# Princic-1837592/julia-raytracer

Measured on AMD Instinct MI355X. Metric: Mrays/s + wall-clock render time, cornellbox 1280×720×256spp, higher is better.
Workload: dtype f32; 1 GPU; cornellbox path 1280x720x256spp; scene=cornellbox, sampler=path, width=1280, height=720, spp=256, bounces=8, batch=256, traversal=near, traversal_requested=auto, bvh=middle, parallelism=1 tile groups x 1 sample ranges + RCCL reduce

## Files before the change

### julia-raytracer_amd/csrc/jt_integrator.h

```cpp
#pragma once

#include <hip/hip_runtime.h>

#include "jt_bsdf.h"
#include "jt_device.h"
#include "jt_launch.h"
#include "jt_scene_eval.h"
#include "jt_traverse.h"

#ifndef JT_FUSED_BSDF
#define JT_FUSED_BSDF 1
#endif

namespace jtk {
using namespace jtd;

template <int F>
__device__ __forceinline__ v3 sample_lights(const DScene& S, v3 position, float rl, float rel, v2 ruv) {
    const int light_id = sample_uniform(S.nlights, rl);
    const DLight l = S.lights[light_id - 1];
    const float* cdf = S.cdf + l.cdf_offset;
    if (l.instance >= 0) {
        const int element = l.nguide ? sample_discrete_guided(cdf, l.ncdf, rel, S.guide_t + l.guide_offset,
                                                              S.guide_a + l.guide_offset, l.nguide, l.guide_scale)
// ... 191 lines not shown
}
template <int F>
__device__ __forceinline__ bool light_hit(const DScene& S, const DParams& P, Path& st, const Hit& h) {
    if (h.hit && light_hit_add<F>(S, st, h)) return false;
    return light_chain_end<F>(S, P, st);
}

#ifndef JT_LIGHT_LEAF_STEP
#define JT_LIGHT_LEAF_STEP 1
#endif
#ifndef JT_CHAIN_TAIL
#define JT_CHAIN_TAIL 2
#endif
__host__ __device__ constexpr bool ft_mesh_kernel(int F) { return mesh_family(F); }
template <bool WIDE, int F>
__host__ __device__ constexpr bool chain_tail() {
    return JT_CHAIN_TAIL && !WIDE && !(F & FT_NOIL) && F != FT_NONE && !ft_mesh_kernel(F);
}
template <bool WIDE, bool OVF, bool NCACHE, int F>
__host__ __device__ constexpr bool chain_leaf_step() {
    return JT_LIGHT_LEAF_STEP && !WIDE && !OVF && !NCACHE && !ft_mesh_kernel(F);
}
template <bool WIDE, bool OVF, bool NCACHE, int F>
__host__ __device__ constexpr bool chain_dinv_once() {
    return JT_CHAIN_TAIL >= 2 && chain_tail<WIDE, F>() && chain_leaf_step<WIDE, OVF, NCACHE, F>();
}

template <bool WIDE, int RING, bool OVF, int COUNT, bool NCACHE, int F, class CountLq>
__device__ __forceinline__ bool light_chain(const DScene& S, const DParams& P, Path& st, Trav& T, int* stack, int pixel,
                                            Counters& cnt, CountLq count_lq) {
    constexpr bool RERUN_LOOP = ft_mesh_kernel(F);
    constexpr bool LEAF = chain_leaf_step<WIDE, OVF, NCACHE, F>(), TAIL = chain_tail<WIDE, F>();
    constexpr bool DINV_ONCE = chain_dinv_once<WIDE, OVF, NCACHE, F>();
    const auto dinv = [&] { T.wdinv = V3(jl_rcp(st.d.x), jl_rcp(st.d.y), jl_rcp(st.d.z)); };
    const auto query = [&] {
        count_lq();
        const int inst = S.lights[st.li].instance;
        if (LEAF) {
            if (!DINV_ONCE) dinv();
            const int negmask = DINV_ONCE && !(F & FT_XFORM) ? T.negmask : neg_mask(st.d, S.order_flip);
            inst_leaf_query<COUNT, F>(S, T, st.o, st.d, T.wdinv, negmask, inst, cnt);
            while (T.nprim > 0) prim_step<COUNT, F>(S, T, cnt);
        } else {
            query_start<WIDE>(S, T, st.o, st.d, inst, stack);
            do {
                node_step_any<WIDE, RING, OVF, COUNT, NCACHE, F>(S, T, stack, pixel, cnt);
                while (T.nprim > 0) prim_step<COUNT, F>(S, T, cnt);
            } while (RERUN_LOOP && rerun_tie<WIDE>(S, T, st.o, st.d, inst, stack));
        }
    };
    if (TAIL) {
        if (DINV_ONCE) {
            dinv();
            if (!(F & FT_XFORM)) T.negmask = neg_mask(st.d, S.order_flip);
        }
        for (;;) {
            do query();
            while (T.h_inst >= 0 && light_hit_add<F>(S, st, query_hit(T)));
            if (light_chain_end<F>(S, P, st)) return true;
            if (st.phase != PH_LIGHT) return false;
        }
    }
    do {
        query();
        if (light_hit<F>(S, P, st, query_hit(T))) return true;
    } while (st.phase == PH_LIGHT);
    return false;
}

struct Aov {
    float* acc;
    float w_;
    int first_;
    int lk_;
    template <int F>
    __device__ __forceinline__ float w() const {
        if (!lane_lds(F)) return w_;
        if (ft_none(F)) return 1.0f / (float)(((reinterpret_cast<const int*>(acc)[11 * BLOCK] - first_) >> lk_) + 1);
        return acc[12 * BLOCK];
    }
};
template <int F>
__device__ __forceinline__ void aov_update(const Aov& a, v3 ta, v3 tn) {
    const float aw = a.w<F>();
    const float omw = 1 - aw;
    float* p = a.acc;
    p[4 * BLOCK] = p[4 * BLOCK] * omw + ta.x * aw;
// ... 206 lines not shown
```

### julia-raytracer_amd/csrc/jt_kernels.h

```cpp
#pragma once

#include <hip/hip_runtime.h>

#include <algorithm>

#include "jt_integrator.h"
#include "jt_launch.h"

namespace jtk {
using namespace jtd;

#ifndef JT_STAMPS
#define JT_STAMPS 0
#endif
#ifndef JT_NODE_REPEAT_NONE
#define JT_NODE_REPEAT_NONE 4
#endif
#ifndef JT_NODE_REPEAT
#define JT_NODE_REPEAT 3
#endif
#ifndef JT_FIRST_POP_NONE
#define JT_FIRST_POP_NONE 1
#endif
#ifndef JT_FIRST_POP
// ... 101 lines not shown
    return JT_ITEM_FIRST_POP == 1 || (JT_ITEM_FIRST_POP == 2 && !WIDE && !ft_none(F));
}
constexpr unsigned ITEM_NONE = 0xffffffffu;

__device__ __forceinline__ int item_pixel(unsigned item, const DParams& P, int tiles_x) {
    const int t = (int)(item >> 6), l = (int)(item & 63u);
    return ((t / tiles_x) * 8 + (l >> 3)) * P.width + (t % tiles_x) * 8 + (l & 7);
}
__host__ __device__ __forceinline__ int item_slot(unsigned item, const DParams& P) {
    const int t = (int)(item >> 6);
    float inv = 1.0f / (float)P.tile_stride;
#if defined(__HIP_DEVICE_COMPILE__)
    inv = __uint_as_float(__builtin_amdgcn_readfirstlane(__float_as_uint(inv)));
#endif
    const int u = (int)((float)(t - P.tile_offset) * inv + 0.5f);
    return u * 64 + (int)(item & 63u);
}
__device__ __forceinline__ float stream_weight(const DParams& P, int s) {
    return 1.0f / (float)(((s - P.first) >> P.lk) + 1);
}

#if JT_STAMPS
#define JT_STAMP(x) x
#else
#define JT_STAMP(x)
#endif

template <int SAMPLER, int RING, bool OVF, int COUNT, int F, bool NCACHE, bool WIDE>
__device__ __forceinline__ void trace_body_items(const DScene& S0, const DParams& P0, int s_begin, int s_end,
                                                 const DAccum& A, int* stack) {
    const DScene& S = S0;
    const DParams& P = P0;
    static_assert(lane_lds(F), "the per-lane item body keeps the lane's sample index in LDS");
    const int lane = threadIdx.x & 63;
    const int oslot = (int)blockIdx.x * BLOCK + (int)threadIdx.x;
    if constexpr ((F & (FT_TEX | FT_ENV)) != 0) {
        for (int k = threadIdx.x; k < 512; k += BLOCK) tex_lut[k] = k < 256 ? S.srgb_lut[k] : S.byte_lut[k - 256];
        __syncthreads();
    }
    Counters cnt{0, 0, 0, 0};
    constexpr bool WC = !ft_none(F);
    unsigned w_paths = 0, w_rays = 0, w_lq = 0;
    __shared__ unsigned wave_cnt[WC ? 1 : (BLOCK / 64) * 4];
    unsigned* const wcnt = wave_cnt + (WC ? 0 : (threadIdx.x >> 6) * 4);
    if (!WC && lane < 3) wcnt[lane] = 0u;
    auto lds_count = [&](int k, bool c) {
        if (c) __hip_atomic_fetch_add(wcnt + k, 1u, __ATOMIC_RELAXED, __HIP_MEMORY_SCOPE_WORKGROUP);
    };
    __shared__ float acc_lds[acc_slots(F) * BLOCK];
    float* acc = acc_lds + threadIdx.x;
    int* const acc_i = reinterpret_cast<int*>(acc);
#if JT_STAMPS
    unsigned long long t_trav = 0, t_shade = 0, n_trav = 0, n_shade = 0, lanes_p = 0, lanes_n = 0, steps_p = 0, steps_n = 0;
    unsigned long long t_hit = 0, t_fin = 0, t_qb = 0, n_phit = 0, n_fin = 0, idle = 0, n_mph = 0, n_mty = 0, n_mid = 0;
    unsigned long long lanes_sh = 0, lanes_hit = 0, t_start = 0, n_start = 0, lanes_start = 0;
#endif
    const int tiles_x = (P.width + 7) / 8, tiles = launch_tiles(P);
    const int kstr = 1 << P.lk;
    const int nq = s_end - s_begin < kstr ? s_end - s_begin : kstr;
    unsigned xcc;
    asm volatile("s_getreg_b32 %0, hwreg(HW_REG_XCC_ID)" : "=s"(xcc));
    int band_k = 0;
    int ut = 0, uq = 0, bnext = 64;
    bool drained = false;
    unsigned item = ITEM_NONE;
    bool next_sample = false;
// ... 56 lines not shown
                            nr = JT_A(normal)[pixel];
                            h = (int)JT_A(hits)[pixel];
                        } else {
                            const size_t o = (size_t)((s - P.first) & (kstr - 1)) * (size_t)JT_A(nslot) +
                                             (size_t)item_slot(item, P);
                            im = JT_A(part_img)[o];
                            al = JT_A(part_alb)[o];
                            nr = JT_A(part_nrm)[o];
                            h = __float_as_int(al.w);
                        }
                    }
                    acc[0] = im.x;
                    acc[BLOCK] = im.y;
                    acc[2 * BLOCK] = im.z;
                    acc[3 * BLOCK] = im.w;
                    acc[4 * BLOCK] = al.x;
                    acc[5 * BLOCK] = al.y;
                    acc[6 * BLOCK] = al.z;
                    acc[7 * BLOCK] = nr.x;
                    acc[8 * BLOCK] = nr.y;
                    acc[9 * BLOCK] = nr.z;
                    acc_i[10 * BLOCK] = h;
                }
            }
            bnext += take;
        }
        next_sample = false;
        if (start) {
            const int sample = acc_i[11 * BLOCK];
            const int pixel = item_pixel(item, P, tiles_x);
            if (!ft_none(F)) acc[12 * BLOCK] = stream_weight(P, sample);
            const DParams& P = karg_params<karg_params_on<SAMPLER, F>()>(P0);
            start_path<F>(P, pixel % P.width, pixel / P.width, pixel, sample, st);
            query_start<WIDE>(S, T, st.o, st.d, -1, stack);
            if (!WC) lds_count(1, true);
            if constexpr (item_first_pop<WIDE, F>()) {
#pragma unroll
                for (int k = 0; k < first_pops<F>(); k++)
                    if (wants_node<WIDE>(T)) node_step_any<WIDE, RING, OVF, COUNT, NCACHE, F>(S, T, stack, oslot, cnt);
            }
        }
        if (WC) w_rays += lane_count(__builtin_amdgcn_ballot_w64(start));
#if JT_STAMPS
        const unsigned long long ts1 = __builtin_amdgcn_s_memtime();
        t_start += ts1 - ts0;
        n_start++;
        lanes_start += lane_count(__builtin_amdgcn_ballot_w64(start));
#endif
        if (__builtin_amdgcn_ballot_w64(item != ITEM_NONE) == 0) break;
        constexpr bool LSTEP = light_steps(SAMPLER, F);
        for (;;) {
            const bool wantp = T.nprim > 0;
            const bool wantn = wants_node<WIDE>(T);
            const bool waiting = query_done<WIDE>(T);
            const int np = lane_count(__builtin_amdgcn_ballot_w64(wantp));
            const int nn = lane_count(__builtin_amdgcn_ballot_w64(wantn));
            int nw = lane_count(__builtin_amdgcn_ballot_w64(waiting));
            const int nb = np + nn;
            if (LSTEP && !S.light_inline) {
                const bool wantl = waiting && st.phase == PH_LIGHT;
                const int nl = lane_count(__builtin_amdgcn_ballot_w64(wantl));
                if (nl > 0 && (nl >= P.light_lanes || nb == 0)) {
                    bool c_lq = false, c_ray = false;
                    if (wantl && rerun_tie<WIDE>(S, T, st.o, st.d, S.lights[st.li].instance, stack)) {
                    } else if (wantl) {
                        if (light_hit<F>(S, P, st, query_hit(T))) {
                            st.phase = PH_FINISH;
                        } else if (st.phase == PH_LIGHT) {
                            if (WC) c_lq = true;
                            else lds_count(2, true);
                            query_start<WIDE>(S, T, st.o, st.d, S.lights[st.li].instance, stack);
                        } else {
                            if (WC) c_ray = true;
                            else lds_count(1, true);
                            query_start<WIDE>(S, T, st.o, st.d, -1, stack);
                        }
                    }
                    if (WC) {
                        w_lq += lane_count(__builtin_amdgcn_ballot_w64(c_lq));
                        w_rays += lane_count(__builtin_amdgcn_ballot_w64(c_ray));
                    }
                    continue;
                }
                nw -= nl;
            }
            if (nb == 0 || nw >= (nb + nw < P.wait_lanes ? nb + nw : P.wait_lanes)) break;
#if JT_STAMPS
            n_trav++;
            idle += 64 - lane_count(__builtin_amdgcn_ballot_w64(item != ITEM_NONE));
            if (np * JT_VOTE_P >= nn * JT_VOTE_N) { steps_p++; lanes_p += np; } else { steps_n++; lanes_n += nn; }
#endif
            if (JT_RAY_FROM_PATH && !(F & FT_XFORM)) {
                T.lo = st.o;
                T.ld = st.d;
            }
            if (np * JT_VOTE_P >= nn * JT_VOTE_N) {
                if (T.nprim > 0) prim_step<COUNT, F>(S, T, cnt);
            } else {
                constexpr int NREP = ft_none(F) ? JT_NODE_REPEAT_NONE : JT_NODE_REPEAT;
#pragma unroll
                for (int k = 0; k < NREP; k++)
                    if (wants_node<WIDE>(T)) node_step_any<WIDE, RING, OVF, COUNT, NCACHE, F>(S, T, stack, oslot, cnt);
            }
        }
#if JT_STAMPS
        const unsigned long long ts2 = __builtin_amdgcn_s_memtime();
        t_trav += ts2 - ts1;
        n_shade++;
        lanes_sh += lane_count(__builtin_amdgcn_ballot_w64(query_done<WIDE>(T)));
        {
            int mid = -1, mt = -1;
            if (query_done<WIDE>(T) && st.phase == PH_SCENE && T.h_inst >= 0) {
                mid = S.inst_shade[T.h_inst].material;
                mt = (F & FT_MAT) ? S.materials[mid].type : (int)M_MATTE;
            }
            if (__builtin_amdgcn_ballot_w64(mt >= 0)) {
                n_mph++;
                lanes_hit += lane_count(__builtin_amdgcn_ballot_w64(mt >= 0));
                for (int ty = 0; ty <= (int)M_GLTFPBR; ty++) n_mty += __builtin_amdgcn_ballot_w64(mt == ty) ? 1u : 0u;
                bool counted = mt < 0;
                for (;;) {
                    const unsigned long long m = __builtin_amdgcn_ballot_w64(!counted);
                    if (!m) break;
                    const int v = __shfl(mid, __ffsll((long long)m) - 1);
                    counted = counted || mid == v;
                    n_mid++;
                }
            }
        }
        unsigned long long ts3 = ts2, ts4 = ts2;
#endif
        constexpr bool LINL = (F & (FT_LINL | FT_NOIL)) != 0;
        {
            const bool tie = query_done<WIDE>(T) && (T.nh & (TIE_SEEN | REF_RERUN)) == TIE_SEEN &&
                             !(LSTEP && st.phase == PH_FINISH);
            if (S.order_flip && __builtin_amdgcn_ballot_w64(tie))
                if (tie) rerun_tie<WIDE>(S, T, st.o, st.d, SAMPLER == 1 && !LINL && st.phase == PH_LIGHT ? S.lights[st.li].instance : -1, stack);
        }
        bool c_path = false, c_lq = false, c_ray = false;
        unsigned n_inl = 0;
        if (query_done<WIDE>(T)) {
            const DParams& P = karg_params<karg_params_on<SAMPLER, F>()>(P0);
            const DScene SL = shade_scene_lds<NCACHE, RING, OVF, F>(S0);
            const DScene& S = NCACHE ? shade_scene<karg_scene<NCACHE, F>()>(S0) : SL;
            bool alive = true;
            const bool light = SAMPLER == 1 && !LINL && st.phase == PH_LIGHT;
            bool done;
            if (LSTEP && st.phase == PH_FINISH) done = true;
            else if (light) done = light_hit<F>(S, P, st, query_hit(T));
            else if (SAMPLER == 2) done = naive_hit<F>(S, P, st, query_hit(T), aov, cnt.shades);
            else done = path_hit<F>(S, P, st, query_hit(T), aov, cnt.shades);
            bool chained = false;
            if (SAMPLER == 1 && !done && st.phase == PH_LIGHT && chains_inline(F, S)) {
                unsigned nlq = 0;
                chained = true;
                done = light_chain<WIDE, RING, OVF, COUNT, NCACHE, F>(S, P, st, T, stack, oslot, cnt, [&] {
                    if (WC) nlq++;
                    else lds_count(2, true);
                });
                if (WC) n_inl += nlq;
            }
#if JT_STAMPS
            ts3 = __builtin_amdgcn_s_memtime();
            n_phit++;
#endif
            if (done) {
                if (WC) c_path = true;
                else lds_count(0, true);
                v3 radiance = st.radiance<F>();
                if (!all_finite(radiance)) radiance = V3(0, 0, 0);
// ... 12 lines not shown
                if (hit || env) acc_i[10 * BLOCK] += 1;
                alive = false;
                T.sp = -1;
                const int sample = acc_i[11 * BLOCK];
                if (sample + kstr >= JT_SE) {
                    const int pixel = item_pixel(item, P, tiles_x);
                    const float4 im = make_float4(acc[0], acc[BLOCK], acc[2 * BLOCK], acc[3 * BLOCK]);
                    if (P.lk == 0) {
                        JT_A(image)[pixel] = im;
                        JT_A(albedo)[pixel] = make_float4(acc[4 * BLOCK], acc[5 * BLOCK], acc[6 * BLOCK], 0.0f);
                        JT_A(normal)[pixel] = make_float4(acc[7 * BLOCK], acc[8 * BLOCK], acc[9 * BLOCK], 0.0f);
                        JT_A(hits)[pixel] = (long long)acc_i[10 * BLOCK];
                    } else {
                        const size_t o = (size_t)((sample - P.first) & (kstr - 1)) * (size_t)JT_A(nslot) +
                                         (size_t)item_slot(item, P);
                        JT_A(part_img)[o] = im;
                        JT_A(part_alb)[o] = make_float4(acc[4 * BLOCK], acc[5 * BLOCK], acc[6 * BLOCK], __int_as_float(acc_i[10 * BLOCK]));
                        JT_A(part_nrm)[o] = make_float4(acc[7 * BLOCK], acc[8 * BLOCK], acc[9 * BLOCK], 0.0f);
                    }
                    item = ITEM_NONE;
                } else {
                    acc_i[11 * BLOCK] = sample + kstr;
                    next_sample = true;
                }
            }
#if JT_STAMPS
            ts4 = __builtin_amdgcn_s_memtime();
            if (__builtin_amdgcn_ballot_w64(done)) n_fin++;
#endif
            if (alive) {
                if (SAMPLER == 1 && !LINL && st.phase == PH_LIGHT) {
                    if (WC) c_lq = true;
                    else lds_count(2, true);
                    query_start<WIDE>(S, T, st.o, st.d, S.lights[st.li].instance, stack);
                } else {
                    if (WC) c_ray = true;
                    else lds_count(1, true);
                    if (SAMPLER == 1 && chain_dinv_once<WIDE, OVF, NCACHE, F>() && __builtin_amdgcn_ballot_w64(!chained) == 0)
                        query_restart<F>(S, T, st.o, st.d, stack);
                    else query_start<WIDE>(S, T, st.o, st.d, -1, stack);
                }
#pragma unroll
                for (int k = 0; k < first_pops<F>(); k++)
                    if (wants_node<WIDE>(T)) node_step_any<WIDE, RING, OVF, COUNT, NCACHE, F>(S, T, stack, oslot, cnt);
            }
        }
#if JT_STAMPS
        const unsigned long long ts5 = __builtin_amdgcn_s_memtime();
        t_shade += ts5 - ts2;
        t_hit += ts3 - ts2;
        t_fin += ts4 - ts3;
        t_qb += ts5 - ts4;
#endif
        if (WC) {
            w_paths += lane_count(__builtin_amdgcn_ballot_w64(c_path));
            w_lq += lane_count(__builtin_amdgcn_ballot_w64(c_lq));
            w_rays += lane_count(__builtin_amdgcn_ballot_w64(c_ray));
            if (SAMPLER == 1 && chains_inline(F, S)) w_lq += __builtin_amdgcn_readfirstlane(wave_sum(n_inl));
        }
    }
#if JT_STAMPS
    if (lane == 0) {
        unsigned long long* dbg = A.counters + 8;
        const unsigned long long v[24] = {t_trav, t_shade, n_trav,  n_shade, lanes_p, lanes_n,  steps_p, steps_n,
                                          0,      t_hit,   t_fin,   t_qb,    0,       n_phit,   n_fin,   idle,
                                          n_mph,  n_mty,   n_mid,   lanes_sh, lanes_hit, t_start, n_start, lanes_start};
        for (int k = 0; k < 24; k++) atomicAdd(dbg + k, v[k]);
    }
#endif
    const unsigned wv[3] = {w_paths, w_rays, w_lq};
    unsigned v[7] = {0u, 0u, 0u, cnt.nodes, cnt.instances, cnt.prims, COUNT ? cnt.shades : 0u};
#pragma unroll
    for (int k = 0; k < 7; k++) {
// ... 11 lines not shown
#if JT_WAVES > 0
#define JT_WAVES_PER_EU __attribute__((amdgpu_waves_per_eu(JT_WAVES, JT_WAVES)))
#define JT_WAVES_PER_EU_F(F) \
    __attribute__((amdgpu_waves_per_eu(ft_none(F) ? JT_WAVES_NONE : JT_WAVES, ft_none(F) ? JT_WAVES_NONE : JT_WAVES)))
#else
#define JT_WAVES_PER_EU
#define JT_WAVES_PER_EU_F(F)
#endif

__device__ __forceinline__ DScene blob_scene(const DScene& S, const uint4* blob) {
    DScene L = S;
    L.nodes = reinterpret_cast<const DNode*>(blob + S.o_nodes);
    L.wnodes = reinterpret_cast<const DWide*>(blob + S.o_wnodes);
    L.prims = reinterpret_cast<const float4*>(blob + S.o_prims);
    L.inst_trav = reinterpret_cast<const DInstTrav*>(blob + S.o_inst_trav);
    L.inst_blas = reinterpret_cast<const int4*>(blob + S.o_inst_blas);
    L.inst_shade = reinterpret_cast<const DInstShade*>(blob + S.o_inst_shade);
    L.shapes = reinterpret_cast<const DShape*>(blob + S.o_shapes);
    L.pos = reinterpret_cast<const float4*>(blob + S.o_pos);
    L.nrm = reinterpret_cast<const float4*>(blob + S.o_nrm);
    L.tc = reinterpret_cast<const float2*>(blob + S.o_tc);
    L.col = reinterpret_cast<const float4*>(blob + S.o_col);
    L.elems = reinterpret_cast<const int4*>(blob + S.o_elems);
    L.enrm = reinterpret_cast<const float4*>(blob + S.o_enrm);
    L.enrm_id = reinterpret_cast<const float4*>(blob + S.o_enrm_id);
    L.materials = reinterpret_cast<const DMaterial*>(blob + S.o_materials);
    L.lights = reinterpret_cast<const DLight*>(blob + S.o_lights);
    L.light_hit = reinterpret_cast<const int4*>(blob + S.o_light_hit);
    L.light_elems = reinterpret_cast<const float4*>(blob + S.o_light_elems);
    L.cdf = reinterpret_cast<const float*>(blob + S.o_cdf);
    return L;
}

template <int SAMPLER, int RING, bool OVF, int COUNT, int F, bool WIDE>
__global__ __launch_bounds__(BLOCK) JT_WAVES_PER_EU void trace_kernel(DScene S, DParams P, int s_begin, int s_end, DAccum A) {
    __shared__ int lds_stack[RING * BLOCK];
    trace_body_items<SAMPLER, RING, OVF, COUNT, F, true, WIDE>(S, P, s_begin, s_end, A, lds_stack + threadIdx.x);
}

template <int SAMPLER, int RING, bool OVF, int COUNT, int F, bool WIDE>
__global__ __launch_bounds__(BLOCK) JT_WAVES_PER_EU_F(F) void trace_kernel_lds(DScene S, DParams P, int s_begin, int s_end, DAccum A) {
    extern __shared__ uint4 dyn_lds[];
    uint4* blob = dyn_lds + lds_stack_bytes(OVF, RING, S.stack_need) / 16;
    for (int k = threadIdx.x; k < S.blob_n16; k += BLOCK) blob[k] = S.blob[k];
    __syncthreads();
    const DScene L = blob_scene(S, blob);
    trace_body_items<SAMPLER, RING, OVF, COUNT, F, false, WIDE>(L, P, s_begin, s_end, A, reinterpret_cast<int*>(dyn_lds) + threadIdx.x);
}

template <int SAMPLER, int RING, bool OVF, int COUNT, int F, bool LDSK, bool WIDE>
hipError_t launch_t(const DScene& S, const DParams& P, int s0, int s1, const DAccum& A, hipStream_t st, int cus) {
    const long long units = (long long)launch_tiles(P) * std::min(s1 - s0, 1 << P.lk);
    const int want = (int)std::min<long long>((units + BLOCK / 64 - 1) / (BLOCK / 64), 1 << 30);
    if (want == 0) return hipSuccess;
    int per_cu = 0;
    hipError_t e;
    if constexpr (LDSK) {
        if (S.blob_n16 > 0) {
        const size_t lds = lds_stack_bytes(OVF, RING, S.stack_need) + (size_t)S.blob_n16 * 16;
        const void* k = (const void*)trace_kernel_lds<SAMPLER, RING, OVF, COUNT, F, WIDE>;
        if ((e = hipFuncSetAttribute(k, hipFuncAttributeMaxDynamicSharedMemorySize, (int)lds)) != hipSuccess) return e;
        if (hipOccupancyMaxActiveBlocksPerMultiprocessor(&per_cu, k, BLOCK, lds) != hipSuccess || per_cu < 1) per_cu = 1;
        const int nwg = std::min(want, std::min(per_cu, 8) * cus);
        hipLaunchKernelGGL((trace_kernel_lds<SAMPLER, RING, OVF, COUNT, F, WIDE>), dim3(nwg), dim3(BLOCK), lds, st, S, P, s0, s1, A);
        return hipGetLastError();
        }
    }
    const void* k = (const void*)trace_kernel<SAMPLER, RING, OVF, COUNT, F, WIDE>;
    if (hipOccupancyMaxActiveBlocksPerMultiprocessor(&per_cu, k, BLOCK, 0) != hipSuccess || per_cu < 1) per_cu = 1;
    const int nwg = std::min(want, std::min(per_cu, 8) * cus);
    hipLaunchKernelGGL((trace_kernel<SAMPLER, RING, OVF, COUNT, F, WIDE>), dim3(nwg), dim3(BLOCK), 0, st, S, P, s0, s1, A);
    return hipGetLastError();
}

template <int ID, int SAMPLER, int COUNT>
hipError_t launch_cfg(const DScene& S, const DParams& P, int s0, int s1, const DAccum& A, hipStream_t st, int cus) {
    using C = LaunchConfig<ID>;
    return launch_t<SAMPLER, C::ring, C::ovf, COUNT, C::feat, C::lds, C::wide>(S, P, s0, s1, A, st, cus);
// ... 4 lines not shown
```

### julia-raytracer_amd/csrc/jt_push.h

```cpp
#pragma once

#if defined(__HIPCC__) || defined(__CUDACC__)
#define JT_PUSH_HD __host__ __device__ inline
#else
#define JT_PUSH_HD inline
#endif

namespace jtk {

constexpr int PUSH_SLOTS = 4;
constexpr unsigned PUSH_T_INST = 1u, PUSH_SNAP_NONE = 63u << 24;

struct PushPlan {
    int npush;
    int first, step;
    unsigned tag;
    bool leaf;
    int slot[PUSH_SLOTS];
    unsigned value[PUSH_SLOTS];
};

JT_PUSH_HD PushPlan push_plan(unsigned meta, int start, unsigned type, bool blas, int negmask, int sp) {
    PushPlan p;
    const bool internal = (meta >> 24) != 0;
    const int num = (int)(meta & 0xffffu);
    const bool neg = ((negmask >> (int)((meta >> 16) & 3u)) & 1) != 0;
    p.npush = internal ? 2 : blas ? 0 : num;
    p.first = internal ? (neg ? start + 1 : start) : start + num - 1;
    p.step = internal && !neg ? 1 : -1;
    p.tag = (internal ? type << 30 : PUSH_T_INST << 30) | PUSH_SNAP_NONE;
    p.leaf = blas && !internal;
    const int last = (p.npush > 1 ? p.npush : 1) - 1;
    const unsigned e0 = p.tag | (unsigned)p.first;
    for (int j = 0; j < PUSH_SLOTS; j++) {
        const int k = j < last ? j : last;
        p.slot[j] = sp + k;
        p.value[j] = e0 + (unsigned)(p.step * k);
    }
    return p;
}

}
```

### julia-raytracer_amd/csrc/jt_traverse.h

```cpp
#pragma once

#include <hip/hip_runtime.h>

#include "jt_device.h"
#include "jt_launch.h"
#include "jt_push.h"

#ifndef JT_CHILD_PRETEST
#define JT_CHILD_PRETEST 1
#endif

namespace jtk {
using namespace jtd;


struct Hit {
    int inst, elem;
    float u, v, t;
    bool hit;
};
struct Counters {
    unsigned nodes, instances, prims, shades;
};

struct Trav {
    v3 wo, wd, wdinv;
    v3 lo, ld, ldinv;
    float tmax;
    int sp;
    int low;
    int inst_space;
    int negmask;
    int cur_inst, cur_kind;
    int prim, nprim;
    int h_inst, h_elem;
    float h_u, h_v;
    int nh;
    unsigned nxt;
};

#ifndef JT_TIE_RERUN
#define JT_TIE_RERUN 1
#endif
constexpr int TIE_SEEN = 1 << 8, REF_RERUN = 1 << 9, NH_COUNT = 63;
__device__ __forceinline__ int query_flip(const DScene& S, const Trav& T) { return (T.nh & REF_RERUN) ? 0 : S.order_flip; }
__device__ __forceinline__ void hit_count(Trav& T, float t) {
    T.nh = (T.nh + ((T.nh & NH_COUNT) < NH_COUNT ? 1 : 0)) | (JT_TIE_RERUN && t == T.tmax ? TIE_SEEN : 0);
}

__device__ __forceinline__ int neg_mask(v3 d, int flip) {
    return ((d.x < 0 ? 1 : 0) | (d.y < 0 ? 2 : 0) | (d.z < 0 ? 4 : 0)) ^ flip;
}

__device__ __forceinline__ void world_ray(const DScene& S, Trav& T) {
    T.lo = T.wo;
    T.ld = T.wd;
    T.ldinv = T.wdinv;
    T.negmask = neg_mask(T.wd, query_flip(S, T));
    T.inst_space = 0;
}

__device__ __forceinline__ Hit query_hit(const Trav& T) {
    return Hit{T.h_inst, T.h_elem, T.h_u, T.h_v, T.tmax, T.h_inst >= 0};
}

__device__ __forceinline__ bool query_busy(const Trav& T) { return T.sp > 0 || T.nprim > 0; }
template <bool WIDE>
__device__ __forceinline__ bool wants_node(const Trav& T) {
    return T.nprim == 0 && (T.sp > 0 || (WIDE && T.nxt != W_EMPTY));
}
template <bool WIDE>
__device__ __forceinline__ bool query_done(const Trav& T) {
    return (T.sp | T.nprim) == 0 && (!WIDE || T.nxt == W_EMPTY);
}

__device__ __forceinline__ void query_ray(Trav& T, v3 o, v3 d) {
    T.wo = o;
    T.wd = d;
    T.wdinv = V3(jl_rcp(d.x), jl_rcp(d.y), jl_rcp(d.z));
    T.lo = o;
    T.ld = d;
    T.ldinv = T.wdinv;
}
__device__ __forceinline__ void query_reset(Trav& T, int nh) {
    T.tmax = __builtin_inff();
    T.nh = nh;
    T.h_inst = -1;
    T.h_elem = -1;
    T.h_u = 0;
    T.h_v = 0;
    T.nprim = 0;
    T.prim = 0;
    T.cur_inst = -1;
    T.cur_kind = KIND_TRI;
    T.inst_space = 0;
}
__device__ __forceinline__ void query_begin(const DScene& S, Trav& T, v3 o, v3 d, unsigned root, int* stack, int rerun = 0) {
    query_ray(T, o, d);
    query_reset(T, rerun);
    T.negmask = neg_mask(d, rerun ? 0 : S.order_flip);
    stack[0] = (int)root;
    T.sp = 1;
    T.low = 0;
    T.nxt = W_EMPTY;
}
__device__ __forceinline__ void query_begin_wide(const DScene& S, Trav& T, v3 o, v3 d, unsigned root_word, int rerun = 0) {
    query_ray(T, o, d);
    query_reset(T, rerun);
    T.negmask = neg_mask(d, rerun ? 0 : S.order_flip);
    T.sp = 0;
    T.low = 0;
    T.nxt = root_word;
}
constexpr unsigned WROOT_SCENE = 0u;
__device__ __forceinline__ unsigned wroot_instance(int inst) { return W_LEAF | W_INST | (unsigned)inst; }
template <bool WIDE>
__device__ __forceinline__ void query_start(const DScene& S, Trav& T, v3 o, v3 d, int inst, int* stack, int rerun = 0) {
    if (WIDE) query_begin_wide(S, T, o, d, inst < 0 ? WROOT_SCENE : wroot_instance(inst), rerun);
    else query_begin(S, T, o, d, inst < 0 ? ((T_TLAS << 30) | SNAP_NONE) : ((T_INST << 30) | SNAP_NONE | (unsigned)inst), stack, rerun);
}
template <int F>
__device__ __forceinline__ void query_restart(const DScene& S, Trav& T, v3 o, v3 d, int* stack) {
    T.wo = o;
    T.wd = d;
    T.lo = o;
    T.ld = d;
    T.ldinv = T.wdinv;
    query_reset(T, 0);
    if (F & FT_XFORM) T.negmask = neg_mask(d, S.order_flip);
    stack[0] = (int)((T_TLAS << 30) | SNAP_NONE);
    T.sp = 1;
    T.low = 0;
    T.nxt = W_EMPTY;
}
constexpr int INST_LEAF_ROOT = 1 << 30;
template <bool WIDE>
__device__ __forceinline__ bool rerun_tie(const DScene& S, Trav& T, v3 o, v3 d, int inst, int* stack) {
    if (!JT_TIE_RERUN || (T.nh & (TIE_SEEN | REF_RERUN)) != TIE_SEEN || S.order_flip == 0) return false;
    if (inst >= 0 && (S.inst_blas[inst].w & INST_LEAF_ROOT)) return false;
    query_start<WIDE>(S, T, o, d, inst, stack, REF_RERUN);
    return true;
}

template <bool XF>
__device__ __forceinline__ void enter_instance(const DScene& S, Trav& T, unsigned inst, const int4& ib) {
    if (!XF || ib.y) {
        if (XF && T.inst_space) world_ray(S, T);
    } else {
        const DInstTrav it = S.inst_trav[inst];
        const fr3 inv = frame_from(it.i0, it.i1, it.i2);
        T.lo = transform_point(inv, T.wo);
        T.ld = transform_vector(inv, T.wd);
        T.ldinv = V3(jl_rcp(T.ld.x), jl_rcp(T.ld.y), jl_rcp(T.ld.z));
        T.negmask = neg_mask(T.ld, query_flip(S, T));
        T.inst_space = 1;
    }
    T.cur_inst = (int)inst;
    T.cur_kind = ib.z;
}

template <int F>
__device__ __forceinline__ void tri_pair(const DScene& S, Trav& T, int k) {
    const float4* r = S.prims + 5 * (T.prim + (k >> 1));
    const float4 r0 = r[0], r1 = r[1], r2 = r[2], r3 = r[3], r4 = r[4];
    const PrimHit p1 = intersect_triangle_pre(T.lo, T.ld, ray_eps, V3(r0.x, r0.z, r1.x), V3(r1.z, r2.x, r2.z),
                                              V3(r3.x, r3.z, r4.x));
    const PrimHit p2 = intersect_triangle_pre(T.lo, T.ld, ray_eps, V3(r0.y, r0.w, r1.y), V3(r1.w, r2.y, r2.w),
                                              V3(r3.y, r3.w, r4.y));
    if (tri_hit_before(p1, T.tmax)) {
        hit_count(T, p1.t);
        T.h_inst = T.cur_inst;
        T.h_elem = __float_as_int(r4.z);
        T.h_u = p1.u;
        T.h_v = p1.v;
        T.tmax = p1.t;
    }
    if (T.nprim >= k + 2 && tri_hit_before(p2, T.tmax)) {
        hit_count(T, p2.t);
        T.h_inst = T.cur_inst;
        T.h_elem = __float_as_int(r4.w);
        T.h_u = p2.u;
        T.h_v = p2.v;
        T.tmax = p2.t;
    }
}
template <int COUNT, int F>
__device__ __forceinline__ void prim_step(const DScene& S, Trav& T, Counters& cnt) {
// ... 26 lines not shown
}

template <int RING, bool OVF>
__device__ __forceinline__ void st_push(const DScene& S, Trav& T, int* stack, int pixel, unsigned e) {
    if (OVF) {
        if (T.sp - T.low == S.ring) {
            S.ovf[(size_t)pixel * S.ovf_stride + T.low] = stack[(T.low & (S.ring - 1)) * BLOCK];
            T.low += 1;
        }
        stack[(T.sp & (S.ring - 1)) * BLOCK] = (int)e;
    } else {
        stack[T.sp * BLOCK] = (int)e;
    }
    T.sp += 1;
}
template <int RING, bool OVF>
__device__ __forceinline__ unsigned st_pop(const DScene& S, Trav& T, const int* stack, int pixel) {
    T.sp -= 1;
    if (OVF) {
        const unsigned r = (unsigned)__hip_atomic_load(stack + (T.sp & (S.ring - 1)) * BLOCK, __ATOMIC_RELAXED,
                                                       __HIP_MEMORY_SCOPE_WORKGROUP);
        if (T.sp < T.low) {
            T.low = T.sp;
            return (unsigned)S.ovf[(size_t)pixel * S.ovf_stride + T.sp];
        }
        return r;
    }
    return (unsigned)stack[T.sp * BLOCK];
}

template <int RING, bool OVF, int COUNT, bool NCACHE, int F>
__device__ __forceinline__ void node_step(const DScene& S, Trav& T, int* stack, int pixel, Counters& cnt) {
    constexpr bool XF = (F & FT_XFORM) != 0;
    const unsigned e = st_pop<RING, OVF>(S, T, stack, pixel);
    unsigned type = e >> 30, idx = e & IDX_MASK;
    if (type == T_INST) {
        if (COUNT) cnt.instances++;
        const int4 ib = S.inst_blas[idx];
        enter_instance<XF>(S, T, idx, ib);
        type = T_BLAS;
        idx = (unsigned)ib.x;
    } else if (XF && type == T_TLAS && T.inst_space) {
        world_ray(S, T);
    }
    const bool blas = type == T_BLAS;
    if (COUNT) cnt.nodes++;
    const unsigned snap = (e >> 24) & 63u;
    float4 nb;
    if (NCACHE) {
        nb = S.nodes[idx].b;
        __asm__("" : "+v"(nb.x), "+v"(nb.y), "+v"(nb.z), "+v"(nb.w));
        if (snap == 63u || snap != (unsigned)(T.nh & NH_COUNT))
            if (!intersect_bbox(T.lo, T.ldinv, ray_eps, T.tmax, S.nodes[idx].a, nb)) return;
    } else {
        const DNode nd = S.nodes[idx];
        if (!intersect_bbox(T.lo, T.ldinv, ray_eps, T.tmax, nd.a, nd.b)) return;
        nb = nd.b;
    }
    const unsigned meta = __float_as_uint(nb.w);
    const int start = __float_as_int(nb.z);
    const int num = (int)(meta & 0xffffu);
    if (!OVF && !(JT_CHILD_PRETEST && NCACHE)) {
        const PushPlan p = push_plan(meta, start, type, blas, T.negmask, T.sp);
#pragma unroll
        for (int j = 0; j < PUSH_SLOTS; j++) stack[p.slot[j] * BLOCK] = (int)p.value[j];
        T.sp += p.npush;
        T.prim = p.leaf ? start : T.prim;
        T.nprim = p.leaf ? num : T.nprim;
        return;
    }
    if (meta >> 24) {
        const int axis = (int)((meta >> 16) & 0xffu);
        const bool neg = (T.negmask >> axis) & 1;
        const unsigned tag = type << 30 | SNAP_NONE;
        const unsigned c_second = (unsigned)(neg ? start + 1 : start), c_first = (unsigned)(neg ? start : start + 1);
        if (JT_CHILD_PRETEST && NCACHE) {
            const DNode n0 = S.nodes[c_second];
            const DNode n1 = S.nodes[c_first];
            const bool k0 = intersect_bbox(T.lo, T.ldinv, ray_eps, T.tmax, n0.a, n0.b);
            const bool k1 = intersect_bbox(T.lo, T.ldinv, ray_eps, T.tmax, n1.a, n1.b);
            if (COUNT) cnt.nodes += (k0 ? 0 : 1) + (k1 ? 0 : 1);
            const unsigned ptag = type << 30 | (unsigned)(T.nh & NH_COUNT) << 24;
            if (k0) st_push<RING, OVF>(S, T, stack, pixel, ptag | c_second);
            if (k1) st_push<RING, OVF>(S, T, stack, pixel, ptag | c_first);
        } else {
            st_push<RING, OVF>(S, T, stack, pixel, tag | c_second);
            st_push<RING, OVF>(S, T, stack, pixel, tag | c_first);
        }
    } else if (!blas) {
        for (int k = num - 1; k >= 0; k--)
            st_push<RING, OVF>(S, T, stack, pixel, (T_INST << 30) | SNAP_NONE | (unsigned)(start + k));
    } else {
        T.prim = start;
        T.nprim = num;

// ... 66 lines not shown
            if (rest) st_push<RING, OVF>(S, T, stack, pixel, (e & ~(15u << 24)) | rest << 24);
            if (XF && T.inst_space && idx < (unsigned)S.tlas_wnodes) world_ray(S, T);
            w = reinterpret_cast<const unsigned*>(S.wnodes + idx)[12 + wide_slot((e >> 28) & 7u, __builtin_ctz(m))];
            if ((w & (W_LEAF | W_INST)) == W_LEAF) {
                wide_take<F>(T, w);
                return;
            }
        } else {
            w = W_LEAF | W_INST | ((e >> 24) & 3u) << 28 | idx;
        }
    } else {
        T.nxt = W_EMPTY;
    }
    if (w & W_LEAF) {
        const unsigned inst = w & W_START, n1 = (w >> 28) & 3u;
        if (n1) st_push<RING, OVF>(S, T, stack, pixel, W_LEAF | (n1 - 1u) << 24 | (inst + 1u));
        if (COUNT) cnt.instances++;
        const int4 ib = S.inst_blas[inst];
        enter_instance<XF>(S, T, inst, ib);
        w = (unsigned)ib.x;
    }
    wide_visit<RING, OVF, COUNT, F>(S, T, stack, pixel, cnt, w);
}
template <bool WIDE, int RING, bool OVF, int COUNT, bool NCACHE, int F>
__device__ __forceinline__ void node_step_any(const DScene& S, Trav& T, int* stack, int pixel, Counters& cnt) {
    if (WIDE) node_step_wide<RING, OVF, COUNT, F>(S, T, stack, pixel, cnt);
    else node_step<RING, OVF, COUNT, NCACHE, F>(S, T, stack, pixel, cnt);
}

template <int COUNT, int F>
__device__ __forceinline__ void inst_leaf_query(const DScene& S, Trav& T, v3 o, v3 d, v3 dinv, int negmask, int inst,
                                                Counters& cnt) {
    constexpr bool XF = (F & FT_XFORM) != 0;
    T.wo = o;
    T.wd = d;
    T.wdinv = dinv;
    T.lo = o;
    T.ld = d;
    T.ldinv = dinv;
    query_reset(T, 0);
    T.negmask = negmask;
    T.sp = 0;
    T.low = 0;
    T.nxt = W_EMPTY;
    if (COUNT) cnt.instances++;
    const int4 ib = S.inst_blas[inst];
    enter_instance<XF>(S, T, (unsigned)inst, ib);
    if (COUNT) cnt.nodes++;
    const DNode nd = S.nodes[ib.x];
    const bool pass = intersect_bbox(T.lo, T.ldinv, ray_eps, T.tmax, nd.a, nd.b);
    T.prim = pass ? __float_as_int(nd.b.z) : 0;
    T.nprim = pass ? (int)(__float_as_uint(nd.b.w) & 0xffffu) : 0;
}

}
```

Before: 12520 Mrays/s.

## Pre-bake BVH node push metadata in LDS to simplify traversal push plan

At kernel start, each BVH node copied into LDS is rewritten so that its start/meta fields hold a precomputed stack tag, push count, axis and leaf flag. The traversal step then derives the child push values with a short baked plan (using v_sad_u32) instead of the general push_plan decode. An extra negmask bit (bit 8) is ORed in so the baked axis-set value always reads as 'no flip'. This aims to cut ALU work per node visit, at the cost of a per-block baking pass with an extra barrier. It also adds a consistency risk: every query start path must pass the push bit.

```diff
diff --git a/julia-raytracer_amd/csrc/jt_integrator.h b/julia-raytracer_amd/csrc/jt_integrator.h
--- a/julia-raytracer_amd/csrc/jt_integrator.h
+++ b/julia-raytracer_amd/csrc/jt_integrator.h
@@ -247,27 +247,28 @@
     constexpr bool RERUN_LOOP = ft_mesh_kernel(F);
     constexpr bool LEAF = chain_leaf_step<WIDE, OVF, NCACHE, F>(), TAIL = chain_tail<WIDE, F>();
     constexpr bool DINV_ONCE = chain_dinv_once<WIDE, OVF, NCACHE, F>();
+    constexpr int PB = push_bit(node_baked<OVF, NCACHE, WIDE, F>());
     const auto dinv = [&] { T.wdinv = V3(jl_rcp(st.d.x), jl_rcp(st.d.y), jl_rcp(st.d.z)); };
     const auto query = [&] {
         count_lq();
         const int inst = S.lights[st.li].instance;
         if (LEAF) {
             if (!DINV_ONCE) dinv();
-            const int negmask = DINV_ONCE && !(F & FT_XFORM) ? T.negmask : neg_mask(st.d, S.order_flip);
+            const int negmask = DINV_ONCE && !(F & FT_XFORM) ? T.negmask : neg_mask(st.d, S.order_flip | PB);
             inst_leaf_query<COUNT, F>(S, T, st.o, st.d, T.wdinv, negmask, inst, cnt);
             while (T.nprim > 0) prim_step<COUNT, F>(S, T, cnt);
         } else {
-            query_start<WIDE>(S, T, st.o, st.d, inst, stack);
+            query_start<WIDE>(S, T, st.o, st.d, inst, stack, 0, PB);
             do {
                 node_step_any<WIDE, RING, OVF, COUNT, NCACHE, F>(S, T, stack, pixel, cnt);
                 while (T.nprim > 0) prim_step<COUNT, F>(S, T, cnt);
-            } while (RERUN_LOOP && rerun_tie<WIDE>(S, T, st.o, st.d, inst, stack));
+            } while (RERUN_LOOP && rerun_tie<WIDE>(S, T, st.o, st.d, inst, stack, PB));
         }
     };
     if (TAIL) {
         if (DINV_ONCE) {
             dinv();
-            if (!(F & FT_XFORM)) T.negmask = neg_mask(st.d, S.order_flip);
+            if (!(F & FT_XFORM)) T.negmask = neg_mask(st.d, S.order_flip | PB);
         }
         for (;;) {
             do query();
diff --git a/julia-raytracer_amd/csrc/jt_kernels.h b/julia-raytracer_amd/csrc/jt_kernels.h
--- a/julia-raytracer_amd/csrc/jt_kernels.h
+++ b/julia-raytracer_amd/csrc/jt_kernels.h
@@ -157,6 +157,7 @@
     const DScene& S = S0;
     const DParams& P = P0;
     static_assert(lane_lds(F), "the per-lane item body keeps the lane's sample index in LDS");
+    constexpr int PB = push_bit(node_baked<OVF, NCACHE, WIDE, F>());
     const int lane = threadIdx.x & 63;
     const int oslot = (int)blockIdx.x * BLOCK + (int)threadIdx.x;
     if constexpr ((F & (FT_TEX | FT_ENV)) != 0) {
@@ -279,7 +280,7 @@
             if (!ft_none(F)) acc[12 * BLOCK] = stream_weight(P, sample);
             const DParams& P = karg_params<karg_params_on<SAMPLER, F>()>(P0);
             start_path<F>(P, pixel % P.width, pixel / P.width, pixel, sample, st);
-            query_start<WIDE>(S, T, st.o, st.d, -1, stack);
+            query_start<WIDE>(S, T, st.o, st.d, -1, stack, 0, PB);
             if (!WC) lds_count(1, true);
             if constexpr (item_first_pop<WIDE, F>()) {
 #pragma unroll
@@ -309,18 +310,18 @@
                 const int nl = lane_count(__builtin_amdgcn_ballot_w64(wantl));
                 if (nl > 0 && (nl >= P.light_lanes || nb == 0)) {
                     bool c_lq = false, c_ray = false;
-                    if (wantl && rerun_tie<WIDE>(S, T, st.o, st.d, S.lights[st.li].instance, stack)) {
+                    if (wantl && rerun_tie<WIDE>(S, T, st.o, st.d, S.lights[st.li].instance, stack, PB)) {
                     } else if (wantl) {
                         if (light_hit<F>(S, P, st, query_hit(T))) {
                             st.phase = PH_FINISH;
                         } else if (st.phase == PH_LIGHT) {
                             if (WC) c_lq = true;
                             else lds_count(2, true);
-                            query_start<WIDE>(S, T, st.o, st.d, S.lights[st.li].instance, stack);
+                            query_start<WIDE>(S, T, st.o, st.d, S.lights[st.li].instance, stack, 0, PB);
                         } else {
                             if (WC) c_ray = true;
                             else lds_count(1, true);
-                            query_start<WIDE>(S, T, st.o, st.d, -1, stack);
+                            query_start<WIDE>(S, T, st.o, st.d, -1, stack, 0, PB);
                         }
                     }
                     if (WC) {
@@ -382,7 +383,7 @@
             const bool tie = query_done<WIDE>(T) && (T.nh & (TIE_SEEN | REF_RERUN)) == TIE_SEEN &&
                              !(LSTEP && st.phase == PH_FINISH);
             if (S.order_flip && __builtin_amdgcn_ballot_w64(tie))
-                if (tie) rerun_tie<WIDE>(S, T, st.o, st.d, SAMPLER == 1 && !LINL && st.phase == PH_LIGHT ? S.lights[st.li].instance : -1, stack);
+                if (tie) rerun_tie<WIDE>(S, T, st.o, st.d, SAMPLER == 1 && !LINL && st.phase == PH_LIGHT ? S.lights[st.li].instance : -1, stack, PB);
         }
         bool c_path = false, c_lq = false, c_ray = false;
         unsigned n_inl = 0;
@@ -461,13 +462,13 @@
                 if (SAMPLER == 1 && !LINL && st.phase == PH_LIGHT) {
                     if (WC) c_lq = true;
                     else lds_count(2, true);
-                    query_start<WIDE>(S, T, st.o, st.d, S.lights[st.li].instance, stack);
+                    query_start<WIDE>(S, T, st.o, st.d, S.lights[st.li].instance, stack, 0, PB);
                 } else {
                     if (WC) c_ray = true;
                     else lds_count(1, true);
                     if (SAMPLER == 1 && chain_dinv_once<WIDE, OVF, NCACHE, F>() && __builtin_amdgcn_ballot_w64(!chained) == 0)
-                        query_restart<F>(S, T, st.o, st.d, stack);
-                    else query_start<WIDE>(S, T, st.o, st.d, -1, stack);
+                        query_restart<F>(S, T, st.o, st.d, stack, PB);
+                    else query_start<WIDE>(S, T, st.o, st.d, -1, stack, 0, PB);
                 }
 #pragma unroll
                 for (int k = 0; k < first_pops<F>(); k++)
@@ -545,6 +546,17 @@
     return L;
 }
 
+__device__ __forceinline__ void bake_nodes(const DScene& S, uint4* blob) {
+    uint4* const nodes = blob + S.o_nodes;
+    const int nnodes = (S.o_wnodes - S.o_nodes) >> 1;
+    for (int k = threadIdx.x; k < nnodes; k += BLOCK) {
+        uint4& b = nodes[2 * k + 1];
+        const BakedNode bn = bake_node(b.w, (int)b.z, k < S.tlas_nnodes ? T_TLAS : T_BLAS);
+        b.z = bn.e0;
+        b.w = bn.meta;
+    }
+}
+
 template <int SAMPLER, int RING, bool OVF, int COUNT, int F, bool WIDE>
 __global__ __launch_bounds__(BLOCK) JT_WAVES_PER_EU void trace_kernel(DScene S, DParams P, int s_begin, int s_end, DAccum A) {
     __shared__ int lds_stack[RING * BLOCK];
@@ -557,6 +569,10 @@
     uint4* blob = dyn_lds + lds_stack_bytes(OVF, RING, S.stack_need) / 16;
     for (int k = threadIdx.x; k < S.blob_n16; k += BLOCK) blob[k] = S.blob[k];
     __syncthreads();
+    if constexpr (node_baked<OVF, false, WIDE, F>()) {
+        bake_nodes(S, blob);
+        __syncthreads();
+    }
     const DScene L = blob_scene(S, blob);
     trace_body_items<SAMPLER, RING, OVF, COUNT, F, false, WIDE>(L, P, s_begin, s_end, A, reinterpret_cast<int*>(dyn_lds) + threadIdx.x);
 }
diff --git a/julia-raytracer_amd/csrc/jt_push.h b/julia-raytracer_amd/csrc/jt_push.h
--- a/julia-raytracer_amd/csrc/jt_push.h
+++ b/julia-raytracer_amd/csrc/jt_push.h
@@ -40,4 +40,51 @@
     return p;
 }
 
+constexpr unsigned BAKE_AXIS_SET = 3u;
+constexpr int BAKE_MASK_BIT = 8;
+constexpr unsigned BAKE_LEAF = 1u << 27;
+
+struct BakedNode {
+    unsigned e0, meta;
+};
+JT_PUSH_HD BakedNode bake_node(unsigned meta, int start, unsigned level) {
+    const bool internal = (meta >> 24) != 0;
+    const bool blas = level != 0u;
+    const unsigned num = meta & 0xffffu;
+    const unsigned tag = (internal ? level << 30 : PUSH_T_INST << 30) | PUSH_SNAP_NONE;
+    const unsigned npush = internal ? 2u : blas ? 0u : (num < (unsigned)PUSH_SLOTS ? num : (unsigned)PUSH_SLOTS);
+    const unsigned last = (npush > 1u ? npush : 1u) - 1u;
+    BakedNode b;
+    b.e0 = internal || !blas ? tag | (unsigned)start : (unsigned)start;
+    b.meta = num | (internal ? (meta >> 16) & 3u : BAKE_AXIS_SET) << 16 | npush << 24 | (!internal && blas ? BAKE_LEAF : 0u) |
+             last << 28 | (last ? 1u : 0u) << 30;
+    return b;
 }
+JT_PUSH_HD unsigned add_absdiff(unsigned a, unsigned b, unsigned c) {
+#if defined(__HIP_DEVICE_COMPILE__)
+    unsigned r;
+    __asm__("v_sad_u32 %0, %1, %2, %3" : "=v"(r) : "v"(a), "v"(b), "v"(c));
+    return r;
+#else
+    return c + (a > b ? a - b : b - a);
+#endif
+}
+JT_PUSH_HD PushPlan push_plan_baked(unsigned e0, unsigned meta, int negmask, int sp) {
+    PushPlan p;
+    p.npush = (int)((meta >> 24) & 7u);
+    p.first = 0;
+    p.step = 0;
+    p.tag = 0u;
+    p.leaf = (meta & BAKE_LEAF) != 0;
+    const unsigned neg = ((unsigned)negmask >> ((meta >> 16) & 3u)) & 1u;
+    const unsigned last = (meta >> 28) & 3u;
+    const unsigned nlast = last * neg;
+    for (int j = 0; j < PUSH_SLOTS; j++) {
+        const unsigned k = j == 1 ? (meta >> 30) & 1u : (unsigned)j < last ? (unsigned)j : last;
+        p.slot[j] = sp + (int)k;
+        p.value[j] = j == 0 ? e0 + nlast : add_absdiff(nlast, k, e0);
+    }
+    return p;
+}
+
+}
diff --git a/julia-raytracer_amd/csrc/jt_traverse.h b/julia-raytracer_amd/csrc/jt_traverse.h
--- a/julia-raytracer_amd/csrc/jt_traverse.h
+++ b/julia-raytracer_amd/csrc/jt_traverse.h
@@ -43,20 +43,34 @@
 #define JT_TIE_RERUN 1
 #endif
 constexpr int TIE_SEEN = 1 << 8, REF_RERUN = 1 << 9, NH_COUNT = 63;
-__device__ __forceinline__ int query_flip(const DScene& S, const Trav& T) { return (T.nh & REF_RERUN) ? 0 : S.order_flip; }
+__device__ __forceinline__ int query_flip(const DScene& S, const Trav& T, int pb = 0) {
+    return ((T.nh & REF_RERUN) ? 0 : S.order_flip) | pb;
+}
 __device__ __forceinline__ void hit_count(Trav& T, float t) {
     T.nh = (T.nh + ((T.nh & NH_COUNT) < NH_COUNT ? 1 : 0)) | (JT_TIE_RERUN && t == T.tmax ? TIE_SEEN : 0);
 }
 
+#ifndef JT_NODE_BAKE
+#define JT_NODE_BAKE 1
+#endif
+#ifndef JT_NODE_READ16
+#define JT_NODE_READ16 0
+#endif
+template <bool OVF, bool NCACHE, bool WIDE, int F>
+__host__ __device__ constexpr bool node_baked() {
+    return JT_NODE_BAKE && !OVF && !NCACHE && !WIDE && ft_none(F);
+}
+__host__ __device__ constexpr int push_bit(bool baked) { return baked ? BAKE_MASK_BIT : 0; }
+
 __device__ __forceinline__ int neg_mask(v3 d, int flip) {
     return ((d.x < 0 ? 1 : 0) | (d.y < 0 ? 2 : 0) | (d.z < 0 ? 4 : 0)) ^ flip;
 }
 
-__device__ __forceinline__ void world_ray(const DScene& S, Trav& T) {
+__device__ __forceinline__ void world_ray(const DScene& S, Trav& T, int pb = 0) {
     T.lo = T.wo;
     T.ld = T.wd;
     T.ldinv = T.wdinv;
-    T.negmask = neg_mask(T.wd, query_flip(S, T));
+    T.negmask = neg_mask(T.wd, query_flip(S, T, pb));
     T.inst_space = 0;
 }
 
@@ -95,10 +109,11 @@
     T.cur_kind = KIND_TRI;
     T.inst_space = 0;
 }
-__device__ __forceinline__ void query_begin(const DScene& S, Trav& T, v3 o, v3 d, unsigned root, int* stack, int rerun = 0) {
+__device__ __forceinline__ void query_begin(const DScene& S, Trav& T, v3 o, v3 d, unsigned root, int* stack, int rerun = 0,
+                                            int pb = 0) {
     query_ray(T, o, d);
     query_reset(T, rerun);
-    T.negmask = neg_mask(d, rerun ? 0 : S.order_flip);
+    T.negmask = neg_mask(d, (rerun ? 0 : S.order_flip) | pb);
     stack[0] = (int)root;
     T.sp = 1;
     T.low = 0;
@@ -115,19 +130,20 @@
 constexpr unsigned WROOT_SCENE = 0u;
 __device__ __forceinline__ unsigned wroot_instance(int inst) { return W_LEAF | W_INST | (unsigned)inst; }
 template <bool WIDE>
-__device__ __forceinline__ void query_start(const DScene& S, Trav& T, v3 o, v3 d, int inst, int* stack, int rerun = 0) {
+__device__ __forceinline__ void query_start(const DScene& S, Trav& T, v3 o, v3 d, int inst, int* stack, int rerun = 0,
+                                            int pb = 0) {
     if (WIDE) query_begin_wide(S, T, o, d, inst < 0 ? WROOT_SCENE : wroot_instance(inst), rerun);
-    else query_begin(S, T, o, d, inst < 0 ? ((T_TLAS << 30) | SNAP_NONE) : ((T_INST << 30) | SNAP_NONE | (unsigned)inst), stack, rerun);
+    else query_begin(S, T, o, d, inst < 0 ? ((T_TLAS << 30) | SNAP_NONE) : ((T_INST << 30) | SNAP_NONE | (unsigned)inst), stack, rerun, pb);
 }
 template <int F>
-__device__ __forceinline__ void query_restart(const DScene& S, Trav& T, v3 o, v3 d, int* stack) {
+__device__ __forceinline__ void query_restart(const DScene& S, Trav& T, v3 o, v3 d, int* stack, int pb = 0) {
     T.wo = o;
     T.wd = d;
     T.lo = o;
     T.ld = d;
     T.ldinv = T.wdinv;
     query_reset(T, 0);
-    if (F & FT_XFORM) T.negmask = neg_mask(d, S.order_flip);
+    if (F & FT_XFORM) T.negmask = neg_mask(d, S.order_flip | pb);
     stack[0] = (int)((T_TLAS << 30) | SNAP_NONE);
     T.sp = 1;
     T.low = 0;
@@ -135,24 +151,24 @@
 }
 constexpr int INST_LEAF_ROOT = 1 << 30;
 template <bool WIDE>
-__device__ __forceinline__ bool rerun_tie(const DScene& S, Trav& T, v3 o, v3 d, int inst, int* stack) {
+__device__ __forceinline__ bool rerun_tie(const DScene& S, Trav& T, v3 o, v3 d, int inst, int* stack, int pb = 0) {
     if (!JT_TIE_RERUN || (T.nh & (TIE_SEEN | REF_RERUN)) != TIE_SEEN || S.order_flip == 0) return false;
     if (inst >= 0 && (S.inst_blas[inst].w & INST_LEAF_ROOT)) return false;
-    query_start<WIDE>(S, T, o, d, inst, stack, REF_RERUN);
+    query_start<WIDE>(S, T, o, d, inst, stack, REF_RERUN, pb);
     return true;
 }
 
 template <bool XF>
-__device__ __forceinline__ void enter_instance(const DScene& S, Trav& T, unsigned inst, const int4& ib) {
+__device__ __forceinline__ void enter_instance(const DScene& S, Trav& T, unsigned inst, const int4& ib, int pb = 0) {
     if (!XF || ib.y) {
-        if (XF && T.inst_space) world_ray(S, T);
+        if (XF && T.inst_space) world_ray(S, T, pb);
     } else {
         const DInstTrav it = S.inst_trav[inst];
         const fr3 inv = frame_from(it.i0, it.i1, it.i2);
         T.lo = transform_point(inv, T.wo);
         T.ld = transform_vector(inv, T.wd);
         T.ldinv = V3(jl_rcp(T.ld.x), jl_rcp(T.ld.y), jl_rcp(T.ld.z));
-        T.negmask = neg_mask(T.ld, query_flip(S, T));
+        T.negmask = neg_mask(T.ld, query_flip(S, T, pb));
         T.inst_space = 1;
     }
     T.cur_inst = (int)inst;
@@ -245,16 +261,18 @@
 template <int RING, bool OVF, int COUNT, bool NCACHE, int F>
 __device__ __forceinline__ void node_step(const DScene& S, Trav& T, int* stack, int pixel, Counters& cnt) {
     constexpr bool XF = (F & FT_XFORM) != 0;
+    constexpr bool BAKED = node_baked<OVF, NCACHE, false, F>();
+    constexpr int PB = push_bit(BAKED);
     const unsigned e = st_pop<RING, OVF>(S, T, stack, pixel);
     unsigned type = e >> 30, idx = e & IDX_MASK;
     if (type == T_INST) {
         if (COUNT) cnt.instances++;
         const int4 ib = S.inst_blas[idx];
-        enter_instance<XF>(S, T, idx, ib);
+        enter_instance<XF>(S, T, idx, ib, PB);
         type = T_BLAS;
         idx = (unsigned)ib.x;
     } else if (XF && type == T_TLAS && T.inst_space) {
-        world_ray(S, T);
+        world_ray(S, T, PB);
     }
     const bool blas = type == T_BLAS;
     if (COUNT) cnt.nodes++;
@@ -266,7 +284,8 @@
         if (snap == 63u || snap != (unsigned)(T.nh & NH_COUNT))
             if (!intersect_bbox(T.lo, T.ldinv, ray_eps, T.tmax, S.nodes[idx].a, nb)) return;
     } else {
-        const DNode nd = S.nodes[idx];
+        DNode nd = S.nodes[idx];
+        if (JT_NODE_READ16 && BAKED) __asm__("" : "+v"(nd.b.x), "+v"(nd.b.y), "+v"(nd.b.z), "+v"(nd.b.w));
         if (!intersect_bbox(T.lo, T.ldinv, ray_eps, T.tmax, nd.a, nd.b)) return;
         nb = nd.b;
     }
@@ -274,6 +293,16 @@
     const int start = __float_as_int(nb.z);
     const int num = (int)(meta & 0xffffu);
     if (!OVF && !(JT_CHILD_PRETEST && NCACHE)) {
+        if constexpr (BAKED) {
+            const PushPlan p = push_plan_baked((unsigned)start, meta, T.negmask, T.sp);
+            int* const top = stack + T.sp * BLOCK;
+#pragma unroll
+            for (int j = 0; j < PUSH_SLOTS; j++) top[(p.slot[j] - T.sp) * BLOCK] = (int)p.value[j];
+            T.sp += p.npush;
+            T.prim = p.leaf ? start : T.prim;
+            T.nprim = p.leaf ? num : T.nprim;
+            return;
+        }
         const PushPlan p = push_plan(meta, start, type, blas, T.negmask, T.sp);
 #pragma unroll
         for (int j = 0; j < PUSH_SLOTS; j++) stack[p.slot[j] * BLOCK] = (int)p.value[j];
@@ -406,6 +435,7 @@
 __device__ __forceinline__ void inst_leaf_query(const DScene& S, Trav& T, v3 o, v3 d, v3 dinv, int negmask, int inst,
                                                 Counters& cnt) {
     constexpr bool XF = (F & FT_XFORM) != 0;
+    constexpr int PB = push_bit(node_baked<false, false, false, F>());
     T.wo = o;
     T.wd = d;
     T.wdinv = dinv;
@@ -419,7 +449,7 @@
     T.nxt = W_EMPTY;
     if (COUNT) cnt.instances++;
     const int4 ib = S.inst_blas[inst];
-    enter_instance<XF>(S, T, (unsigned)inst, ib);
+    enter_instance<XF>(S, T, (unsigned)inst, ib, PB);
     if (COUNT) cnt.nodes++;
     const DNode nd = S.nodes[ib.x];
     const bool pass = intersect_bbox(T.lo, T.ldinv, ray_eps, T.tmax, nd.a, nd.b);
```

Result: faster. 13290 Mrays/s (median of 6 runs) (+6.1%).
